# jopohl/urh

Hardware: AMD Instinct MI355X
Metric: Msamples/s IQ->bits (1 GiB complex64 2-FSK per GPU, qad materialised, compact outputs copied to the host) (higher is better)
Workload: dtype f32

## Files before the change

### urh_amd/csrc/costas.hip

```cpp
#include <hip/hip_runtime.h>

#include <algorithm>
#include <atomic>
#include <math.h>
#include <string.h>
#include <type_traits>

#include "cmul.hpp"
#include "common.hpp"
#include "launchers.hpp"
#include "glibc_sincosf.h"

namespace urh {

struct CostasArgs {
    const void *iq; int64_t n; float *out;
    float noise_sqrd, alpha, beta, scale, shift;
    int loop_order;
    int warm;
    const float *d_noise = nullptr;
};
struct CostasState { float freq, phase; };
struct CostasArgsSh : CostasArgs {
    const void *halo_end;
    int64_t origin;
    int64_t lo;
    int64_t start1;
};
template <bool SH> using CostasArgsT = typename std::conditional<SH, CostasArgsSh, CostasArgs>::type;

__device__ __forceinline__ float costas_clamp(float x) {
    float r = (x > 1.0f) ? 1.0f : x;
    r = (x < -1.0f) ? -1.0f : r;
    return r;
}

template <int DT> struct CostasLoad;
template <> struct CostasLoad<URHGPU_DT_F32> { static __device__ __forceinline__ float2 at(const void *p, int64_t i) { return ((const float2 *)p)[i]; } };
template <> struct CostasLoad<URHGPU_DT_I8> { static __device__ __forceinline__ float2 at(const void *p, int64_t i) { const char2 v = ((const char2 *)p)[i]; return make_float2((float)v.x, (float)v.y); } };
template <> struct CostasLoad<URHGPU_DT_U8> { static __device__ __forceinline__ float2 at(const void *p, int64_t i) { const uchar2 v = ((const uchar2 *)p)[i]; return make_float2((float)v.x, (float)v.y); } };
template <> struct CostasLoad<URHGPU_DT_I16> { static __device__ __forceinline__ float2 at(const void *p, int64_t i) { const short2 v = ((const short2 *)p)[i]; return make_float2((float)v.x, (float)v.y); } };
template <> struct CostasLoad<URHGPU_DT_U16> { static __device__ __forceinline__ float2 at(const void *p, int64_t i) { const ushort2 v = ((const ushort2 *)p)[i]; return make_float2((float)v.x, (float)v.y); } };

template <class A>
__device__ __forceinline__ A costas_device_noise(const A &a_in) {
    A a = a_in;
    if (a.d_noise) a.noise_sqrd = *a.d_noise;
    return a;
}
__device__ __forceinline__ bool costas_gated(float2 sm, const CostasArgs &a) { return sm.x * sm.x + sm.y * sm.y <= a.noise_sqrd; }

template <bool UNIT = false, int ORDER = 0>
__device__ __forceinline__ float costas_step(float2 sm, CostasState &st, float &err, const CostasArgs &a) {
    const int loop_order = ORDER ? ORDER : a.loop_order;
    if (costas_gated(sm, a)) return -4.0f;
    const double two_pi = 2 * 3.14159265358979323846;
    const float real_float = UNIT ? sm.x + 0.0f : (sm.x + a.shift) / a.scale, imag_float = UNIT ? sm.y + 0.0f : (sm.y + a.shift) / a.scale;
    const float2 cur = make_float2(real_float + 0.0f * imag_float, 1.0f * imag_float);
    float sn, cs;
    if (urh_sc_abstop12(st.phase) < 0x42f) urh_sincosf_fast(-st.phase, &sn, &cs);
    else { sn = urh_sinf(-st.phase); cs = urh_cosf(-st.phase); }
    const float2 nco = make_float2(cs + 0.0f * sn, 1.0f * sn);
    const float2 z = cmul(nco, cur);
    if (loop_order == 2) {
        err = z.y * z.x;
    } else if (loop_order == 4) {
        const float f1 = z.x > 0.0f ? 1.0f : -1.0f, f2 = z.y > 0.0f ? 1.0f : -1.0f;
        err = f1 * z.y - f2 * z.x;
    }
    err = costas_clamp(err);
    st.freq += a.beta * err;
    st.phase += st.freq + a.alpha * err;
    while ((double)st.phase > two_pi) st.phase = (float)((double)st.phase - two_pi);
    while ((double)st.phase < -two_pi) st.phase = (float)((double)st.phase + two_pi);
    st.freq = costas_clamp(st.freq);
    if (loop_order == 2) return z.x;
    if (loop_order == 4) return (float)(2.0 * (double)z.x + (double)z.y);
    return 0.0f;
}

template <bool UNIT, int ORDER>
__device__ __forceinline__ float costas_step_bf(float2 sm, CostasState &st, float &err, const CostasArgs &a) {
    static_assert(ORDER == 2 || ORDER == 4, "the serial kernel handles the other orders");
    const double two_pi = 2 * 3.14159265358979323846;
    const CostasState old = st;
    const float old_err = err;
    const bool gated = costas_gated(sm, a);
    const float real_float = UNIT ? sm.x + 0.0f : (sm.x + a.shift) / a.scale, imag_float = UNIT ? sm.y + 0.0f : (sm.y + a.shift) / a.scale;
    const float2 cur = make_float2(real_float + 0.0f * imag_float, 1.0f * imag_float);
    const bool in_range = __builtin_fabsf(old.phase) <= __uint_as_float(0x40C90FDBu);
    float sn, cs;
    urh_sincosf_fast(-old.phase, &sn, &cs);
    const float2 nco = make_float2(cs + 0.0f * sn, 1.0f * sn);
    float2 z;
    z.x = nco.x * cur.x - nco.y * cur.y;
    z.y = nco.x * cur.y + nco.y * cur.x;
    const bool rare = !gated && (!in_range || ((z.x != z.x) & (z.y != z.y)));
    float e;
    if (ORDER == 2) e = z.y * z.x;
    else {
        const float f1 = z.x > 0.0f ? 1.0f : -1.0f, f2 = z.y > 0.0f ? 1.0f : -1.0f;
        e = f1 * z.y - f2 * z.x;
    }
    e = costas_clamp(e);
    float freq = old.freq + a.beta * e;
    float phase = old.phase + (freq + a.alpha * e);
    const double d = (double)phase;
    const float wrapped_down = (float)(d - two_pi), wrapped_up = (float)(d + two_pi);
    phase = (d > two_pi) ? wrapped_down : ((d < -two_pi) ? wrapped_up : phase);
    freq = costas_clamp(freq);
    const float out = (ORDER == 2) ? z.x : (float)(2.0 * (double)z.x + (double)z.y);
    if (__builtin_expect(__builtin_amdgcn_ballot_w64(rare) != 0, 0)) {
        st = old; err = old_err;
        return costas_step<UNIT, ORDER>(sm, st, err, a);
    }
    st.freq = gated ? old.freq : freq;
    st.phase = gated ? old.phase : phase;
    err = gated ? old_err : e;
    return gated ? -4.0f : out;
}

constexpr int kCostasTile = 1024;

template <int DT>
__global__ __launch_bounds__(64) void k_costas(const CostasArgs a_in) {
    const CostasArgs a = costas_device_noise(a_in);
    __shared__ float2 s_x[kCostasTile];
    const int lane = threadIdx.x;
    CostasState st{0.0f, 1.5f};
    float err = 0.0f;
    if (lane == 0 && a.n > 0) a.out[0] = -4.0f;
    for (int64_t base = 0; base < a.n; base += kCostasTile) {
        const int tv = (int)((a.n - base < kCostasTile) ? (a.n - base) : kCostasTile);
        __syncthreads();
        for (int u = lane; u < tv; u += 64) s_x[u] = CostasLoad<DT>::at(a.iq, base + u);
        __syncthreads();
        float mine[kCostasTile / 64];
#pragma unroll 1
        for (int g = 0; g < kCostasTile / 64; ++g) {
            float keep = 0.0f;
#pragma unroll 1
            for (int u = 0; u < 64; ++u) {
                const int k = g * 64 + u;
                if (k >= tv || (base + k) == 0) continue;
                const float o = costas_step<DT == URHGPU_DT_F32>(s_x[k], st, err, a);
                if (u == lane) keep = o;
            }
            mine[g] = keep;
        }
#pragma unroll 1
        for (int g = 0; g < kCostasTile / 64; ++g) {
            const int k = g * 64 + lane;
            if (k < tv && base + k != 0) a.out[base + k] = mine[g];
        }
    }
}

#ifndef URH_COSTAS_CHUNK
#define URH_COSTAS_CHUNK 4096
#endif
constexpr int kChunk = URH_COSTAS_CHUNK;
constexpr int kWarmBackFactor = 16;
constexpr int kCkpt = 256;
constexpr int kNumCkpt = kChunk / kCkpt;
constexpr int kMaxCand = 8;

struct SpecBuffers {
    CostasState *S;
    CostasState *E;
    CostasState *CP;
    uint32_t *map;
    CostasState *T;
    int32_t *run_list;
    int32_t *run_count;
    uint8_t *is_rep;
    int32_t *gidx;
    int32_t *ungated;
    CostasState *resume;
    int32_t *stats;
};
struct CostasCtl {
    int64_t c_from;
    int32_t use_seed;
    float seed_freq;
    int32_t done;
    int32_t rounds;
};
__host__ __device__ __forceinline__ CostasCtl *costas_ctl(const SpecBuffers &b) { return (CostasCtl *)(b.stats + 16); }

__device__ __forceinline__ bool same_state(CostasState a, CostasState b) {
    return __float_as_uint(a.freq) == __float_as_uint(b.freq) && __float_as_uint(a.phase) == __float_as_uint(b.phase);
}
__device__ __forceinline__ int64_t chunk_begin(int64_t c) { return 1 + c * (int64_t)kChunk; }

template <bool SH, class A> __device__ __forceinline__ int64_t chunk_begin_of(const A &a, int64_t c) {
    if constexpr (SH) return a.origin + c * (int64_t)kChunk;
    else return chunk_begin(c);
}
template <int DT, bool SH, class A> __device__ __forceinline__ float2 costas_at(const A &a, int64_t i) {
    if constexpr (SH) return CostasLoad<DT>::at(i < 0 ? a.halo_end : a.iq, i);
    else return CostasLoad<DT>::at(a.iq, i);
}
template <bool SH, class A> __device__ __forceinline__ int64_t walk_floor(const A &a) {
    if constexpr (SH) return a.lo;
    else return 1;
}
template <bool SH, class A> __device__ __forceinline__ int64_t loop_start(const A &a) {
    if constexpr (SH) return a.start1;
    else return 1;
}
template <bool SH, class A> __device__ __forceinline__ bool chunk0_exact(const A &a) {
    if constexpr (SH) return a.origin == 1;
    else return true;
}

template <int DT, int ORDER, bool SH = false, bool DEV = false>
__global__ __launch_bounds__(256) void k_costas_spec(const CostasArgsT<SH> a_in, SpecBuffers b, int64_t n_chunks, int K, int64_t c_from,
                                                      int use_seed, float seed_freq) {
    const CostasArgsT<SH> a = costas_device_noise(a_in);
    if constexpr (DEV) {
        if (costas_ctl(b)->done) return;
        c_from = costas_ctl(b)->c_from; use_seed = costas_ctl(b)->use_seed; seed_freq = costas_ctl(b)->seed_freq;
    }
    const int64_t gid = blockIdx.x * 256ll + threadIdx.x;
    const int64_t c = c_from + gid / K;
    const int k = (int)(gid % K);
    if (c >= n_chunks) return;
    const int64_t s0 = chunk_begin_of<SH>(a, c);
    const float spacing = (a.loop_order == 4) ? 1.57079632679489661923f : 3.14159265358979323846f;
    CostasState st{0.0f, 1.5f + (float)(k - K / 2) * spacing};
    float err = 0.0f;
    int64_t p = s0;
    if (c == 0 && chunk0_exact<SH>(a)) {
        st = CostasState{0.0f, 1.5f};
    } else {
        int ungated = 0;
        const int64_t back = (int64_t)kWarmBackFactor * a.warm;
        const int64_t floor = walk_floor<SH>(a);
        while (p > floor && ungated < a.warm && s0 - p < back) {
            float2 g[8];
#pragma unroll
            for (int j = 0; j < 8; ++j) g[j] = costas_at<DT, SH>(a, (p - 1 - j >= floor) ? p - 1 - j : floor);
#pragma unroll
            for (int j = 0; j < 8; ++j) {
                if (p > floor && ungated < a.warm && s0 - p < back) {
                    --p;
                    if (!costas_gated(g[j], a)) ++ungated;
                }
            }
        }
        if (p == loop_start<SH>(a)) {
            st = CostasState{0.0f, 1.5f};
        } else if (use_seed) {
            st.freq = seed_freq;
        } else {
            float ax = 0.0f, ay = 0.0f;
            float2 prev = costas_at<DT, SH>(a, p);
            bool prev_ok = !costas_gated(prev, a);
            const int64_t wend = (p + 512 < s0) ? p + 512 : s0;
            for (int64_t i0 = p + 1; i0 < wend; i0 += 8) {
                float2 g[8];
#pragma unroll
                for (int j = 0; j < 8; ++j) g[j] = costas_at<DT, SH>(a, (i0 + j < wend) ? i0 + j : wend - 1);
#pragma unroll
                for (int j = 0; j < 8; ++j) {
                    if (i0 + j < wend) {
                        const float2 cur = g[j];
                        const bool ok = !costas_gated(cur, a);
                        if (ok && prev_ok) {
                            const float cr = (cur.x + a.shift) / a.scale, ci = (cur.y + a.shift) / a.scale;
                            const float pr = (prev.x + a.shift) / a.scale, pi = (prev.y + a.shift) / a.scale;
                            float dx = cr * pr + ci * pi, dy = ci * pr - cr * pi;
                            float tx = dx * dx - dy * dy, ty = 2.0f * dx * dy;
                            if (a.loop_order == 4) { const float ux = tx * tx - ty * ty, uy = 2.0f * tx * ty; tx = ux; ty = uy; }
                            ax += tx; ay += ty;
                        }
                        prev = cur; prev_ok = ok;
                    }
                }
            }
            if (ax != 0.0f || ay != 0.0f) st.freq = costas_clamp(atan2f(ay, ax) / (float)a.loop_order);
        }
        {
            constexpr int PF = 4;
            float2 cur[PF];
#pragma unroll
            for (int j = 0; j < PF; ++j) cur[j] = costas_at<DT, SH>(a, (p + j < s0) ? p + j : s0 - 1);
            for (int64_t i = p; i < s0; i += PF) {
                float2 nxt[PF];
#pragma unroll
                for (int j = 0; j < PF; ++j) { const int64_t q = i + PF + j; nxt[j] = costas_at<DT, SH>(a, (q < s0) ? q : s0 - 1); }
#pragma unroll
                for (int j = 0; j < PF; ++j) if (i + j < s0) costas_step_bf<DT == URHGPU_DT_F32, ORDER>(cur[j], st, err, a);
#pragma unroll
                for (int j = 0; j < PF; ++j) cur[j] = nxt[j];
            }
        }
    }
    b.S[c * K + k] = st;
    const int lane = threadIdx.x & 63, base = lane - k;
    bool dup = false;
    for (int j = 0; j < K; ++j) {
        CostasState o;
        o.freq = __shfl(st.freq, base + j); o.phase = __shfl(st.phase, base + j);
        if (j < k && same_state(o, st)) dup = true;
    }
    b.is_rep[c * K + k] = dup ? 0 : 1;
    const unsigned long long m = __ballot(!dup);
    int pos = 0;
    if (lane == __builtin_ctzll(m)) pos = atomicAdd(b.run_count, __builtin_popcountll(m));
    pos = __shfl(pos, __builtin_ctzll(m));
    if (!dup) b.run_list[pos + __builtin_popcountll(m & ((1ull << lane) - 1ull))] = (int32_t)(c * K + k);
}

template <int DT, int ORDER, bool SH = false>
__global__ __launch_bounds__(256) void k_costas_run(const CostasArgsT<SH> a_in, SpecBuffers b, int K) {
    const CostasArgsT<SH> a = costas_device_noise(a_in);
    const int64_t gid = blockIdx.x * 256ll + threadIdx.x;
    if (gid >= *b.run_count) return;
    const int64_t ck = b.run_list[gid];
    const int64_t c = ck / K;
    const int k = (int)(ck % K);
    const int64_t s0 = chunk_begin_of<SH>(a, c);
    const int64_t e0 = (s0 + kChunk < a.n) ? s0 + kChunk : a.n;
    CostasState st = b.S[ck];
    float err = 0.0f;
    int ung = 0;
    constexpr int PF = 4;
    float2 cur[PF];
#pragma unroll
    for (int j = 0; j < PF; ++j) cur[j] = CostasLoad<DT>::at(a.iq, (s0 + j < e0) ? s0 + j : e0 - 1);
    for (int64_t i = s0; i < e0; i += PF) {
        float2 nxt[PF];
#pragma unroll
        for (int j = 0; j < PF; ++j) { const int64_t q = i + PF + j; nxt[j] = CostasLoad<DT>::at(a.iq, (q < e0) ? q : e0 - 1); }
#pragma unroll
        for (int j = 0; j < PF; ++j) {
            if (i + j < e0) {
                if (!costas_gated(cur[j], a)) ++ung;
                costas_step_bf<DT == URHGPU_DT_F32, ORDER>(cur[j], st, err, a);
                const int off = (int)(i + j - s0) + 1;
                if (off % kCkpt == 0 && off < kChunk) b.CP[(c * kNumCkpt + (off / kCkpt - 1)) * K + k] = st;
            }
        }
#pragma unroll
        for (int j = 0; j < PF; ++j) cur[j] = nxt[j];
    }
    b.E[ck] = st;
    if (k == 0) b.ungated[c] = ung;
}

template <bool DEV = false>
__global__ __launch_bounds__(256) void k_costas_map(SpecBuffers b, int64_t n_chunks, int K, int64_t c_from) {
    if constexpr (DEV) {
        if (costas_ctl(b)->done) return;
        c_from = costas_ctl(b)->c_from > 1 ? costas_ctl(b)->c_from : 1;
    }
    const int64_t c = c_from + blockIdx.x * 256ll + threadIdx.x;
    if (c >= n_chunks) return;
    uint32_t m = 0xFFFFFFFFu;
    if (c > 0) {
        for (int k = 0; k < K; ++k) {
            int hit = 0xF;
            if (b.is_rep[(c - 1) * K + k]) {
                const CostasState e = b.E[(c - 1) * K + k];
                for (int q = 0; q < K; ++q) if (same_state(e, b.S[c * K + q])) { hit = q; break; }
            }
            m = (m & ~(0xFu << (4 * k))) | ((uint32_t)hit << (4 * k));
        }
    }
    b.map[c] = m;
}

__device__ __forceinline__ uint32_t map_compose(uint32_t later, uint32_t earlier) {
    uint32_t r = 0;
#pragma unroll
    for (int k = 0; k < 8; ++k) {
        const uint32_t mid = (earlier >> (4 * k)) & 0xFu;
        const uint32_t v = (mid == 0xFu) ? 0xFu : ((later >> (4 * mid)) & 0xFu);
        r |= v << (4 * k);
    }
    return r;
}

constexpr int kStitchBlock = 1024;
template <int DT, int ORDER, bool SH = false, bool DEV = false>
__global__ __launch_bounds__(kStitchBlock) void k_costas_stitch(const CostasArgsT<SH> a_in, SpecBuffers b, int64_t n_chunks, int K, int64_t c_from,
                                                                 int allow_break) {
    const CostasArgsT<SH> a = costas_device_noise(a_in);
    if constexpr (DEV) {
        const int done = costas_ctl(b)->done;
        c_from = costas_ctl(b)->c_from > 1 ? costas_ctl(b)->c_from : 1;
        __syncthreads();
        if (done) return;
    }
    __shared__ uint32_t s_wp[kStitchBlock / 64];
    __shared__ int s_fail, s_cand, s_flags;
    __shared__ CostasState s_T;
    __shared__ long long s_c;
    const int tid = threadIdx.x, lane = tid & 63, wave = tid >> 6;
    int cand = -1;
    CostasState T = *b.resume;
    if (!SH && c_from == 1) { cand = 0; if (tid == 0) { b.T[0] = CostasState{0.0f, 1.5f}; b.gidx[0] = 0; } }
    int n_map = 0, n_ckpt = 0, n_serial = 0;
    int64_t stop_at = n_chunks;
    int64_t c = c_from;
    bool map_failed = false;
    bool stop = false;
    while (c < n_chunks && !stop) {
        while (cand >= 0 && c < n_chunks) {
            constexpr int Q = 4;
            if (tid == 0) s_fail = 0x7fffffff;
            const int64_t cc0 = c + (int64_t)Q * tid;
            uint32_t L[Q];
#pragma unroll
            for (int q = 0; q < Q; ++q) {
                const uint32_t m = (cc0 + q < n_chunks) ? b.map[cc0 + q] : 0xFFFFFFFFu;
                L[q] = q ? map_compose(m, L[q - 1]) : m;
            }
            uint32_t P = L[Q - 1];
#pragma unroll
            for (int o = 1; o < 64; o <<= 1) {
                const uint32_t u = __shfl_up(P, o);
                if (lane >= o) P = map_compose(P, u);
            }
            if (lane == 63) s_wp[wave] = P;
            __syncthreads();
            uint32_t X = 0x76543210u;
            for (int w = 0; w < wave; ++w) X = map_compose(s_wp[w], X);
            const uint32_t before = __shfl_up(P, 1);
            if (lane != 0) X = map_compose(before, X);
            uint32_t g[Q], gp[Q];
#pragma unroll
            for (int q = 0; q < Q; ++q) g[q] = (map_compose(L[q], X) >> (4 * cand)) & 0xFu;
            gp[0] = (X >> (4 * cand)) & 0xFu;
#pragma unroll
            for (int q = 1; q < Q; ++q) gp[q] = g[q - 1];
            CostasState Tl[Q];
            int firstq = Q;
#pragma unroll
            for (int q = Q - 1; q >= 0; --q) {
                const int64_t cc = cc0 + q;
                const bool reach = (gp[q] != 0xFu) && (cc < n_chunks);
                Tl[q] = T;
                if (reach) { Tl[q] = b.E[(cc - 1) * K + gp[q]]; b.T[cc] = Tl[q]; b.gidx[cc] = (g[q] == 0xFu) ? -1 : (int32_t)g[q]; }
                if (reach && g[q] == 0xFu) firstq = q;
            }
            if (firstq < Q) atomicMin(&s_fail, tid * Q + firstq);
            __syncthreads();
            const int fail = s_fail;
            const int64_t left = n_chunks - c;
            const int total = (int)(left < (int64_t)kStitchBlock * Q ? left : (int64_t)kStitchBlock * Q);
            const int pos = (fail == 0x7fffffff) ? total - 1 : fail;
            if (tid == pos / Q) {
                const int qq = pos % Q;
                uint32_t gl = g[0];
                CostasState Ts = Tl[0];
#pragma unroll
                for (int q = 1; q < Q; ++q) if (qq == q) { gl = g[q]; Ts = Tl[q]; }
                s_cand = (int)gl; s_T = Ts;
            }
            __syncthreads();
            if (fail == 0x7fffffff) {
                cand = s_cand;
                n_map += total; c += total;
            } else {
                T = s_T;
                n_map += fail; c += fail; cand = -1; map_failed = true;
            }
            __syncthreads();
        }
        if (c >= n_chunks) break;
        if (wave == 0) {
            bool done = false;
            if (!map_failed) {
                if (lane == 0) { b.T[c] = T; b.gidx[c] = -1; }
                const bool hit = lane < K && same_state(T, b.S[c * K + lane]);
                const unsigned long long m = __ballot(hit);
                if (m) {
                    cand = __builtin_ctzll(m);
                    if (lane == 0) b.gidx[c] = cand;
                    ++n_map; ++c;
                    done = true;
                }
            }
            if (!done) {
                map_failed = false;
                if (b.ungated[c] == 0) { ++n_serial; ++c; done = true; }
            }
            if (!done) {
                const int64_t s0 = chunk_begin_of<SH>(a, c);
                const int64_t e0 = (s0 + kChunk < a.n) ? s0 + kChunk : a.n;
                float err = 0.0f;
                CostasState st = T;
                for (int64_t i = s0; i < e0; ++i) {
                    costas_step_bf<DT == URHGPU_DT_F32, ORDER>(CostasLoad<DT>::at(a.iq, i), st, err, a);
                    const int off = (int)(i - s0) + 1;
                    if (off % kCkpt == 0 && off < kChunk) {
                        const bool hit = lane < K && b.is_rep[c * K + lane] && same_state(st, b.CP[(c * kNumCkpt + (off / kCkpt - 1)) * K + lane]);
                        const unsigned long long m = __ballot(hit);
                        if (m) { cand = __builtin_ctzll(m); break; }
                    }
                }
                if (cand >= 0) { ++n_ckpt; ++c; }
                else {
                    ++n_serial;
                    T = st;
                    if (allow_break && b.ungated[c] >= kChunk / 2 && c + 1 < n_chunks) { stop_at = c + 1; stop = true; }
                    else ++c;
                }
            }
            if (lane == 0) { s_c = c; s_cand = cand; s_T = T; s_flags = (map_failed ? 1 : 0) | (stop ? 2 : 0); }
        }
        __syncthreads();
        c = s_c; cand = s_cand; T = s_T; map_failed = (s_flags & 1) != 0; stop = (s_flags & 2) != 0;
        __syncthreads();
    }
    if (tid == 0) {
        b.stats[0] += n_map; b.stats[1] += n_ckpt; b.stats[2] += n_serial; b.stats[3] = (int32_t)stop_at;
        *b.resume = T;
        if constexpr (SH) b.resume[1] = (cand >= 0) ? b.E[(n_chunks - 1) * K + cand] : T;
        if constexpr (DEV) {
            CostasCtl *ctl = costas_ctl(b);
            if (stop_at < n_chunks) { ctl->c_from = stop_at; ctl->use_seed = 1; ctl->seed_freq = T.freq; ctl->rounds += 1; }
            else ctl->done = 1;
            b.stats[4] = ctl->rounds;
        }
    }
}

template <int DT, int ORDER, bool SH = false>
__global__ __launch_bounds__(256) void k_costas_final(const CostasArgsT<SH> a_in, SpecBuffers b, int64_t n_chunks, int K) {
    const CostasArgsT<SH> a = costas_device_noise(a_in);
    const int64_t gid = blockIdx.x * 256ll + threadIdx.x;
    const int64_t c = gid / kNumCkpt;
    const int j = (int)(gid % kNumCkpt);
    if (c >= n_chunks) return;
    if (gid == 0 && a.n > 0 && chunk0_exact<SH>(a)) a.out[0] = -4.0f;
    const int64_t s0 = chunk_begin_of<SH>(a, c);
    const int64_t e0 = (s0 + kChunk < a.n) ? s0 + kChunk : a.n;
    const int g = b.gidx[c];
    int64_t i0 = s0, i1 = e0;
    CostasState st = b.T[c];
    if (g >= 0) {
        i0 = s0 + (int64_t)j * kCkpt;
        i1 = (i0 + kCkpt < e0) ? i0 + kCkpt : e0;
        if (j > 0) st = b.CP[(c * kNumCkpt + (j - 1)) * K + g];
    } else if (j != 0) return;
    float err = 0.0f;
    constexpr int kTileF = 16;
    int64_t i = i0;
    for (; i + kTileF <= i1; i += kTileF) {
        float2 x[kTileF];
#pragma unroll
        for (int u = 0; u < kTileF; ++u) x[u] = CostasLoad<DT>::at(a.iq, i + u);
        float o[kTileF];
#pragma unroll 1
        for (int u = 0; u < kTileF; ++u) {
            float2 xv = x[0];
#pragma unroll
            for (int q = 1; q < kTileF; ++q) if (u == q) xv = x[q];
            const float ov = costas_step_bf<DT == URHGPU_DT_F32, ORDER>(xv, st, err, a);
#pragma unroll
            for (int q = 0; q < kTileF; ++q) if (u == q) o[q] = ov;
        }
#pragma unroll
        for (int u = 0; u < kTileF; ++u) a.out[i + u] = o[u];
    }
    for (; i < i1; ++i) a.out[i] = costas_step_bf<DT == URHGPU_DT_F32, ORDER>(CostasLoad<DT>::at(a.iq, i), st, err, a);
}

constexpr size_t kCtlSlot = 64;
static_assert(sizeof(CostasCtl) <= kCtlSlot, "control block");
size_t costas_scratch_bytes(int64_t n) {
    const int64_t nc = (std::max<int64_t>(n - 1, 0) + kChunk - 1) / kChunk + 1;
    return (size_t)nc * kMaxCand * sizeof(CostasState) * 2 + (size_t)nc * kNumCkpt * kMaxCand * sizeof(CostasState) +
           (size_t)nc * 4 * 3 + (size_t)nc * sizeof(CostasState) + (size_t)nc * kMaxCand * 5 + 3 * 64 + kCtlSlot + 16 * 256;
}

constexpr int kMaxRounds = 24;
std::atomic<long long> g_costas_host_syncs{0};

static SpecBuffers spec_buffers(void *scratch, int64_t nc, int K) {
    char *p = (char *)scratch;
    auto take = [&](size_t bytes) { char *r = p; p += (bytes + 255) & ~size_t(255); return r; };
    SpecBuffers b;
    b.S = (CostasState *)take((size_t)nc * K * sizeof(CostasState));
    b.E = (CostasState *)take((size_t)nc * K * sizeof(CostasState));
    b.CP = (CostasState *)take((size_t)nc * kNumCkpt * K * sizeof(CostasState));
    b.map = (uint32_t *)take((size_t)nc * 4);
    b.T = (CostasState *)take((size_t)nc * sizeof(CostasState));
    b.ungated = (int32_t *)take((size_t)nc * 4);
    b.gidx = (int32_t *)take((size_t)nc * 4);
    b.run_list = (int32_t *)take((size_t)nc * K * 4);
    b.is_rep = (uint8_t *)take((size_t)nc * K);
    b.run_count = (int32_t *)take(64);
    b.resume = (CostasState *)take(64);
    b.stats = (int32_t *)take(64 + kCtlSlot);
    return b;
}
void costas_scratch_layout(int64_t n, int K, int64_t out3[3]) {
    const int64_t nc = (std::max<int64_t>(n - 1, 0) + kChunk - 1) / kChunk;
    const SpecBuffers b = spec_buffers(nullptr, nc, K);
    out3[0] = (int64_t)costas_scratch_bytes(n);
    out3[1] = (int64_t)(uintptr_t)costas_ctl(b) + (int64_t)sizeof(CostasCtl);
    out3[2] = (int64_t)sizeof(CostasCtl);
}

template <int DT, int ORDER>
static int launch_costas_spec(const CostasArgs &a, void *scratch, urhgpu_ctx *ctx);
template <int DT, int ORDER>
static int launch_costas_dev(const CostasArgs &a, void *scratch, urhgpu_ctx *ctx, int rounds, int32_t *h_stats);

constexpr double kEmptyRoundUs = 25.0, kCostasBaseUs = 1800.0, kCostasUsPerChunk = 0.046, kEmptyRoundsShare = 0.10;
static int costas_auto_rounds(int64_t nc) {
    const double fit = kEmptyRoundsShare * (kCostasBaseUs + kCostasUsPerChunk * (double)nc) / kEmptyRoundUs;
    return (int)std::min<double>(kMaxRounds, std::max<double>(2.0, fit));
}

template <int DT>
static int launch_costas_dt(const CostasArgs &a, void *scratch, urhgpu_ctx *ctx) {
    const bool parallel = (a.loop_order == 2 || a.loop_order == 4) && a.n > 2 * kChunk && scratch != nullptr;
    int32_t *h_stats = ctx->costas_stats_next ? ctx->costas_stats_next : (int32_t *)(ctx->h_counts + 12);
    if (!parallel) {
        hipLaunchKernelGGL(k_costas<DT>, dim3(1), dim3(64), 0, ctx->stream, a);
        memset(h_stats, 0, 24);
        return URHGPU_OK;
    }
    if (ctx->tune_costas_dev_rounds >= 0 || ctx->pipelined) {
        const int rounds = ctx->tune_costas_dev_rounds >= 0 ? ctx->tune_costas_dev_rounds : costas_auto_rounds((a.n - 1 + kChunk - 1) / kChunk);
        return a.loop_order == 4 ? launch_costas_dev<DT, 4>(a, scratch, ctx, rounds, h_stats) : launch_costas_dev<DT, 2>(a, scratch, ctx, rounds, h_stats);
    }
    return a.loop_order == 4 ? launch_costas_spec<DT, 4>(a, scratch, ctx) : launch_costas_spec<DT, 2>(a, scratch, ctx);
}

template <int DT, int ORDER>
static int launch_costas_dev(const CostasArgs &a, void *scratch, urhgpu_ctx *ctx, int rounds, int32_t *h_stats) {
    hipStream_t s = ctx->stream;
    const int K = (a.loop_order == 4) ? 8 : 4;
    const int64_t nc = (a.n - 1 + kChunk - 1) / kChunk;
    SpecBuffers b = spec_buffers(scratch, nc, K);
    URH_HIP(hipMemsetAsync(b.stats, 0, 64 + kCtlSlot, s));
    URH_HIP(hipMemsetAsync(b.resume, 0, 64, s));
    const dim3 g_cand((unsigned)((nc * K + 255) / 256)), g_chunk((unsigned)((nc + 255) / 256));
    for (int round = 0; round <= rounds; ++round) {
        URH_HIP(hipMemsetAsync(b.run_count, 0, 4, s));
        hipLaunchKernelGGL((k_costas_spec<DT, ORDER, false, true>), g_cand, dim3(256), 0, s, a, b, nc, K, (int64_t)0, 0, 0.0f);
        hipLaunchKernelGGL((k_costas_run<DT, ORDER>), g_cand, dim3(256), 0, s, a, b, K);
        hipLaunchKernelGGL(k_costas_map<true>, g_chunk, dim3(256), 0, s, b, nc, K, (int64_t)1);
        hipLaunchKernelGGL((k_costas_stitch<DT, ORDER, false, true>), dim3(1), dim3(kStitchBlock), 0, s, a, b, nc, K, (int64_t)1, round < rounds ? 1 : 0);
    }
    hipLaunchKernelGGL((k_costas_final<DT, ORDER>), dim3((unsigned)((nc * kNumCkpt + 255) / 256)), dim3(256), 0, s, a, b, nc, K);
    URH_HIP(hipGetLastError());
    URH_HIP(hipMemcpyAsync(h_stats, b.stats, 20, hipMemcpyDeviceToHost, s));
    return URHGPU_OK;
}

template <int DT, int ORDER>
static int launch_costas_spec(const CostasArgs &a, void *scratch, urhgpu_ctx *ctx) {
    hipStream_t s = ctx->stream;
    const int K = (a.loop_order == 4) ? 8 : 4;
    const int64_t nc = (a.n - 1 + kChunk - 1) / kChunk;
    SpecBuffers b = spec_buffers(scratch, nc, K);
    URH_HIP(hipMemsetAsync(b.stats, 0, 64, s));
    URH_HIP(hipMemsetAsync(b.resume, 0, 64, s));
    int64_t c_from = 0;
    int use_seed = 0;
    float seed_freq = 0.0f;
    int32_t *h = (int32_t *)(ctx->h_counts + 12);
    int rounds = 0;
    for (int round = 0;; ++round) {
        const int64_t todo = nc - c_from;
        URH_HIP(hipMemsetAsync(b.run_count, 0, 4, s));
        hipLaunchKernelGGL((k_costas_spec<DT, ORDER>), dim3((unsigned)((todo * K + 255) / 256)), dim3(256), 0, s, a, b, nc, K, c_from, use_seed,
                           seed_freq);
        hipLaunchKernelGGL((k_costas_run<DT, ORDER>), dim3((unsigned)((todo * K + 255) / 256)), dim3(256), 0, s, a, b, K);
        hipLaunchKernelGGL(k_costas_map<false>, dim3((unsigned)((todo + 255) / 256)), dim3(256), 0, s, b, nc, K, std::max<int64_t>(c_from, 1));
        hipLaunchKernelGGL((k_costas_stitch<DT, ORDER>), dim3(1), dim3(kStitchBlock), 0, s, a, b, nc, K, std::max<int64_t>(c_from, 1),
                           round < kMaxRounds ? 1 : 0);
        URH_HIP(hipGetLastError());
        URH_HIP(hipMemcpyAsync(h, b.stats, 20, hipMemcpyDeviceToHost, s));
        URH_HIP(hipMemcpyAsync(h + 6, b.resume, 8, hipMemcpyDeviceToHost, s));
        URH_HIP(hipStreamSynchronize(s));
        ++g_costas_host_syncs;
        center_note_wait();
        const int64_t stop_at = h[3];
        if (stop_at >= nc) break;
        c_from = stop_at;
        use_seed = 1;
        memcpy(&seed_freq, h + 6, 4);
        rounds = round + 1;
    }
    h[4] = rounds;
    hipLaunchKernelGGL((k_costas_final<DT, ORDER>), dim3((unsigned)((nc * kNumCkpt + 255) / 256)), dim3(256), 0, s, a, b, nc, K);
    return URHGPU_OK;
}

static int costas_warm(float bandwidth) {
    const double want = 40.0 / std::max(1e-3, std::min(1.0, (double)fabsf(bandwidth)));
    int w = 256;
    while (w < want && w < 8192) w *= 2;
    return w;
}

static int costas_args(const urhgpu_params *p, CostasArgs &a) {
    a.noise_sqrd = p->noise_threshold * p->noise_threshold;
    const float bandwidth = p->costas_loop_bandwidth;
    const float damping = (float)(sqrt(2.0) / 2.0);
    const double den = (1.0 + ((2.0 * (double)damping) * (double)bandwidth)) + (double)(bandwidth * bandwidth);
    a.alpha = (float)(((4.0 * (double)damping) * (double)bandwidth) / den);
    a.beta = (float)(((4.0 * (double)bandwidth) * (double)bandwidth) / den);
    switch (p->dtype) {
        case URHGPU_DT_I8: a.scale = 127.5f; a.shift = 0.5f; break;
        case URHGPU_DT_U8: a.scale = 127.5f; a.shift = -127.5f; break;
        case URHGPU_DT_I16: a.scale = 32767.5f; a.shift = 0.5f; break;
        case URHGPU_DT_U16: a.scale = 65535.0f; a.shift = -32767.5f; break;
        case URHGPU_DT_F32: a.scale = 1.0f; a.shift = 0.0f; break;
        default: return URHGPU_ERR_DTYPE;
    }
    a.warm = costas_warm(bandwidth);
    int order = p->mod_order > 0 ? p->mod_order : (1 << p->bits_per_symbol);
    if (order > 4) order = 4;
    a.loop_order = order;
    return URHGPU_OK;
}

int launch_costas(urhgpu_ctx *ctx, const void *d_iq, int64_t n, const urhgpu_params *p, float *d_qad, void *scratch, const float *d_noise) {
    CostasArgs a;
    a.iq = d_iq; a.n = n; a.out = d_qad; a.d_noise = d_noise;
    URH_TRY(costas_args(p, a));
    switch (p->dtype) {
        case URHGPU_DT_I8: return launch_costas_dt<URHGPU_DT_I8>(a, scratch, ctx);
        case URHGPU_DT_U8: return launch_costas_dt<URHGPU_DT_U8>(a, scratch, ctx);
        case URHGPU_DT_I16: return launch_costas_dt<URHGPU_DT_I16>(a, scratch, ctx);
        case URHGPU_DT_U16: return launch_costas_dt<URHGPU_DT_U16>(a, scratch, ctx);
        default: return launch_costas_dt<URHGPU_DT_F32>(a, scratch, ctx);
    }
}


int64_t costas_halo_samples(const urhgpu_params *p) { return (int64_t)kWarmBackFactor * costas_warm(p->costas_loop_bandwidth); }

constexpr int kSumBlock = 1024;
__global__ __launch_bounds__(kSumBlock) void k_costas_shard_summary(SpecBuffers b, int64_t n_chunks, int K, uint32_t *out) {
    __shared__ uint32_t s_wp[kSumBlock / 64];
    __shared__ unsigned long long s_ung;
    const int tid = threadIdx.x, lane = tid & 63, wave = tid >> 6;
    if (tid == 0) s_ung = 0;
    __syncthreads();
    unsigned long long ung = 0;
    for (int64_t c = tid; c < n_chunks; c += kSumBlock) ung += (uint32_t)b.ungated[c];
    atomicAdd(&s_ung, ung);
    uint32_t R = 0x76543210u;
    constexpr int Q = 4;
    for (int64_t c0 = 1; c0 < n_chunks; c0 += (int64_t)kSumBlock * Q) {
        const int64_t cc0 = c0 + (int64_t)Q * tid;
        uint32_t P = 0x76543210u;
#pragma unroll
        for (int q = 0; q < Q; ++q) if (cc0 + q < n_chunks) P = map_compose(b.map[cc0 + q], P);
#pragma unroll
        for (int o = 1; o < 64; o <<= 1) {
            const uint32_t u = __shfl_up(P, o);
            if (lane >= o) P = map_compose(P, u);
        }
        if (lane == 63) s_wp[wave] = P;
        __syncthreads();
        for (int w = 0; w < kSumBlock / 64; ++w) R = map_compose(s_wp[w], R);
        __syncthreads();
    }
    __syncthreads();
    if (tid < kCostasSummaryBytes / 4) {
        const int64_t last = (n_chunks - 1) * K;
        uint32_t v = 0;
        if (tid < 16) {
            const int k = tid >> 1;
            if (k < K) { const CostasState s = b.S[k]; v = __float_as_uint((tid & 1) ? s.phase : s.freq); }
        } else if (tid < 32) {
            const int k = (tid - 16) >> 1;
            if (k < K && b.is_rep[last + k]) { const CostasState e = b.E[last + k]; v = __float_as_uint((tid & 1) ? e.phase : e.freq); }
        } else if (tid == 32) {
            v = R;
        } else if (tid == 33) {
            for (int k = 0; k < K; ++k) v |= b.is_rep[k] ? (1u << k) : 0u;
        } else if (tid == 34) {
            v = (s_ung == 0) ? 1u : 0u;
        } else if (tid == 35) {
            v = (uint32_t)K;
        } else if (tid < 38) {
            v = (uint32_t)((uint64_t)n_chunks >> (32 * (tid - 36)));
        } else {
            v = (uint32_t)(s_ung >> (32 * (tid - 38)));
        }
        out[tid] = v;
    }
}

__global__ void k_costas_set_state(CostasState *dst, uint32_t freq_bits, uint32_t phase_bits) {
    uint32_t *d = (uint32_t *)dst;
    d[0] = freq_bits; d[1] = phase_bits;
}

static int costas_shard_args(const CostasShard &cs, CostasArgsSh &a, int64_t &nc) {
    a.iq = cs.iq; a.n = cs.n; a.out = cs.out;
    URH_TRY(costas_args(&cs.p, a));
    if (a.loop_order != 2 && a.loop_order != 4) return URHGPU_ERR_UNSUPPORTED;
    a.halo_end = cs.halo_end; a.origin = cs.origin; a.lo = cs.lo; a.start1 = cs.start1;
    nc = (cs.n - cs.origin + kChunk - 1) / kChunk;
    return URHGPU_OK;
}

template <int DT, int ORDER>
static int costas_shard_spec_t(urhgpu_ctx *ctx, const CostasArgsSh &a, int64_t nc, void *scratch, void *d_summary) {
    hipStream_t s = ctx->stream;
    const int K = (ORDER == 4) ? 8 : 4;
    const SpecBuffers b = spec_buffers(scratch, nc, K);
    URH_HIP(hipMemsetAsync(b.stats, 0, 64, s));
    URH_HIP(hipMemsetAsync(b.resume, 0, 64, s));
    URH_HIP(hipMemsetAsync(b.run_count, 0, 4, s));
    const unsigned g = (unsigned)((nc * K + 255) / 256);
    hipLaunchKernelGGL((k_costas_spec<DT, ORDER, true>), dim3(g), dim3(256), 0, s, a, b, nc, K, (int64_t)0, 0, 0.0f);
    hipLaunchKernelGGL((k_costas_run<DT, ORDER, true>), dim3(g), dim3(256), 0, s, a, b, K);
    hipLaunchKernelGGL(k_costas_map<false>, dim3((unsigned)((nc + 255) / 256)), dim3(256), 0, s, b, nc, K, (int64_t)1);
    hipLaunchKernelGGL(k_costas_shard_summary, dim3(1), dim3(kSumBlock), 0, s, b, nc, K, (uint32_t *)d_summary);
    URH_HIP(hipGetLastError());
    return URHGPU_OK;
}

template <int DT, int ORDER>
static int costas_shard_resolve_t(urhgpu_ctx *ctx, const CostasArgsSh &a, int64_t nc, void *scratch, uint32_t freq_bits, uint32_t phase_bits,
                                  void *d_end) {
    hipStream_t s = ctx->stream;
    const int K = (ORDER == 4) ? 8 : 4;
    const SpecBuffers b = spec_buffers(scratch, nc, K);
    hipLaunchKernelGGL(k_costas_set_state, dim3(1), dim3(1), 0, s, b.resume, freq_bits, phase_bits);
    int64_t c_from = 0;
    float seed_freq = 0.0f;
    int32_t *h = (int32_t *)(ctx->h_counts + 12);
    int rounds = 0;
    for (int round = 0;; ++round) {
        if (round > 0) {
            const int64_t todo = nc - c_from;
            URH_HIP(hipMemsetAsync(b.run_count, 0, 4, s));
            hipLaunchKernelGGL((k_costas_spec<DT, ORDER, true>), dim3((unsigned)((todo * K + 255) / 256)), dim3(256), 0, s, a, b, nc, K, c_from, 1,
                               seed_freq);
            hipLaunchKernelGGL((k_costas_run<DT, ORDER, true>), dim3((unsigned)((todo * K + 255) / 256)), dim3(256), 0, s, a, b, K);
            hipLaunchKernelGGL(k_costas_map<false>, dim3((unsigned)((todo + 255) / 256)), dim3(256), 0, s, b, nc, K, c_from);
        }
        hipLaunchKernelGGL((k_costas_stitch<DT, ORDER, true>), dim3(1), dim3(kStitchBlock), 0, s, a, b, nc, K, c_from,
                           round < kMaxRounds ? 1 : 0);
        URH_HIP(hipGetLastError());
        URH_HIP(hipMemcpyAsync(h, b.stats, 20, hipMemcpyDeviceToHost, s));
        URH_HIP(hipMemcpyAsync(h + 6, b.resume, 8, hipMemcpyDeviceToHost, s));
        URH_HIP(hipStreamSynchronize(s));
        ++g_costas_host_syncs;
        center_note_wait();
        const int64_t stop_at = h[3];
        if (stop_at >= nc) break;
        c_from = stop_at;
        memcpy(&seed_freq, h + 6, 4);
        rounds = round + 1;
    }
    h[4] = rounds;
    if (d_end) URH_HIP(hipMemcpyAsync(d_end, b.resume + 1, 8, hipMemcpyDeviceToDevice, s));
    hipLaunchKernelGGL((k_costas_final<DT, ORDER, true>), dim3((unsigned)((nc * kNumCkpt + 255) / 256)), dim3(256), 0, s, a, b, nc, K);
    URH_HIP(hipGetLastError());
    return URHGPU_OK;
}

#define URH_COSTAS_SHARD_DISPATCH(FN, ...)                                                                                       \
    switch (cs.p.dtype) {                                                                                                        \
        case URHGPU_DT_I8: return a.loop_order == 4 ? FN<URHGPU_DT_I8, 4>(__VA_ARGS__) : FN<URHGPU_DT_I8, 2>(__VA_ARGS__);        \
        case URHGPU_DT_U8: return a.loop_order == 4 ? FN<URHGPU_DT_U8, 4>(__VA_ARGS__) : FN<URHGPU_DT_U8, 2>(__VA_ARGS__);        \
        case URHGPU_DT_I16: return a.loop_order == 4 ? FN<URHGPU_DT_I16, 4>(__VA_ARGS__) : FN<URHGPU_DT_I16, 2>(__VA_ARGS__);     \
        case URHGPU_DT_U16: return a.loop_order == 4 ? FN<URHGPU_DT_U16, 4>(__VA_ARGS__) : FN<URHGPU_DT_U16, 2>(__VA_ARGS__);     \
        case URHGPU_DT_F32: return a.loop_order == 4 ? FN<URHGPU_DT_F32, 4>(__VA_ARGS__) : FN<URHGPU_DT_F32, 2>(__VA_ARGS__);     \
        default: return URHGPU_ERR_DTYPE;                                                                                        \
    }

int launch_costas_shard_spec(urhgpu_ctx *ctx, const CostasShard &cs, void *d_summary) {
    CostasArgsSh a;
    int64_t nc = 0;
    URH_TRY(costas_shard_args(cs, a, nc));
    URH_COSTAS_SHARD_DISPATCH(costas_shard_spec_t, ctx, a, nc, cs.scratch, d_summary)
}

int launch_costas_shard_resolve(urhgpu_ctx *ctx, const CostasShard &cs, uint32_t freq_bits, uint32_t phase_bits, void *d_end) {
    CostasArgsSh a;
    int64_t nc = 0;
    URH_TRY(costas_shard_args(cs, a, nc));
    URH_COSTAS_SHARD_DISPATCH(costas_shard_resolve_t, ctx, a, nc, cs.scratch, freq_bits, phase_bits, d_end)
}
#undef URH_COSTAS_SHARD_DISPATCH

__global__ __launch_bounds__(256) void k_test_sincosf_fast(unsigned long long *mismatches) {
    unsigned long long bad = 0;
    for (uint64_t u = blockIdx.x * 256ull + threadIdx.x; u < 2ull * 0x42f00000ull; u += (uint64_t)gridDim.x * 256ull) {
        const uint32_t bits = (u < 0x42f00000ull) ? (uint32_t)u : ((uint32_t)(u - 0x42f00000ull) | 0x80000000u);
        const float y = __uint_as_float(bits);
        float sn, cs;
        urh_sincosf_fast(y, &sn, &cs);
        if (__float_as_uint(sn) != __float_as_uint(urh_sinf(y)) || __float_as_uint(cs) != __float_as_uint(urh_cosf(y))) ++bad;
    }
    if (bad) atomicAdd(mismatches, bad);
}
void launch_test_sincosf_fast(unsigned long long *d_mismatches, hipStream_t s) {
    hipLaunchKernelGGL(k_test_sincosf_fast, dim3(256 * 32), dim3(256), 0, s, d_mismatches);
}

}
```

Measured before the change: 496,700.

## Split Costas warm-up backward walk and frequency seed across the K hypothesis lanes

Result: no change. 496,500 (-0.0%).

```diff
diff --git a/urh_amd/csrc/costas.hip b/urh_amd/csrc/costas.hip
--- a/urh_amd/csrc/costas.hip
+++ b/urh_amd/csrc/costas.hip
@@ -214,6 +214,21 @@
     else return true;
 }
 
+__device__ __forceinline__ int nth_set_bit(uint64_t m, int n) {
+    int pos = 0;
+#pragma unroll
+    for (int w = 32; w; w >>= 1) {
+        const int low = __builtin_popcountll(m & ((1ull << w) - 1ull));
+        const bool skip = n > low;
+        n = skip ? n - low : n; m = skip ? m >> w : m; pos = skip ? pos + w : pos;
+    }
+    return pos;
+}
+template <int DT> __device__ __forceinline__ float2 seed_scaled(float2 sm, float shift, float inv_scale) {
+    if constexpr (DT == URHGPU_DT_F32) return sm;
+    else return make_float2((sm.x + shift) * inv_scale, (sm.y + shift) * inv_scale);
+}
+
 template <int DT, int ORDER, bool SH = false, bool DEV = false>
 __global__ __launch_bounds__(256) void k_costas_spec(const CostasArgsT<SH> a_in, SpecBuffers b, int64_t n_chunks, int K, int64_t c_from,
                                                       int use_seed, float seed_freq) {
@@ -226,6 +241,8 @@
     const int64_t c = c_from + gid / K;
     const int k = (int)(gid % K);
     if (c >= n_chunks) return;
+    constexpr int KK = (ORDER == 4) ? 8 : 4;
+    const int lane = threadIdx.x & 63, base = lane - k;
     const int64_t s0 = chunk_begin_of<SH>(a, c);
     const float spacing = (a.loop_order == 4) ? 1.57079632679489661923f : 3.14159265358979323846f;
     CostasState st{0.0f, 1.5f + (float)(k - K / 2) * spacing};
@@ -237,16 +254,25 @@
         int ungated = 0;
         const int64_t back = (int64_t)kWarmBackFactor * a.warm;
         const int64_t floor = walk_floor<SH>(a);
-        while (p > floor && ungated < a.warm && s0 - p < back) {
+        const int64_t lim = (s0 - back > floor) ? s0 - back : floor;
+        while (p > lim && ungated < a.warm) {
+            const int room = (p - lim > 8 * KK) ? 8 * KK : (int)(p - lim);
             float2 g[8];
 #pragma unroll
-            for (int j = 0; j < 8; ++j) g[j] = costas_at<DT, SH>(a, (p - 1 - j >= floor) ? p - 1 - j : floor);
+            for (int j = 0; j < 8; ++j) { const int t = j * KK + k; g[j] = costas_at<DT, SH>(a, p - 1 - ((t < room) ? t : room - 1)); }
+            uint64_t seen = 0;
 #pragma unroll
             for (int j = 0; j < 8; ++j) {
-                if (p > floor && ungated < a.warm && s0 - p < back) {
-                    --p;
-                    if (!costas_gated(g[j], a)) ++ungated;
-                }
+                const unsigned long long bal = __ballot(j * KK + k < room && !costas_gated(g[j], a));
+                seen |= ((bal >> base) & ((1ull << KK) - 1ull)) << (j * KK);
+            }
+            const int have = __builtin_popcountll(seen), need = a.warm - ungated;
+            if (have < need) {
+                ungated += have;
+                p -= room;
+            } else {
+                ungated = a.warm;
+                p -= 1 + nth_set_bit(seen, need);
             }
         }
         if (p == loop_start<SH>(a)) {
@@ -255,30 +281,36 @@
             st.freq = seed_freq;
         } else {
             float ax = 0.0f, ay = 0.0f;
-            float2 prev = costas_at<DT, SH>(a, p);
-            bool prev_ok = !costas_gated(prev, a);
             const int64_t wend = (p + 512 < s0) ? p + 512 : s0;
-            for (int64_t i0 = p + 1; i0 < wend; i0 += 8) {
-                float2 g[8];
-#pragma unroll
-                for (int j = 0; j < 8; ++j) g[j] = costas_at<DT, SH>(a, (i0 + j < wend) ? i0 + j : wend - 1);
-#pragma unroll
-                for (int j = 0; j < 8; ++j) {
-                    if (i0 + j < wend) {
-                        const float2 cur = g[j];
-                        const bool ok = !costas_gated(cur, a);
-                        if (ok && prev_ok) {
-                            const float cr = (cur.x + a.shift) / a.scale, ci = (cur.y + a.shift) / a.scale;
-                            const float pr = (prev.x + a.shift) / a.scale, pi = (prev.y + a.shift) / a.scale;
-                            float dx = cr * pr + ci * pi, dy = ci * pr - cr * pi;
-                            float tx = dx * dx - dy * dy, ty = 2.0f * dx * dy;
-                            if (a.loop_order == 4) { const float ux = tx * tx - ty * ty, uy = 2.0f * tx * ty; tx = ux; ty = uy; }
-                            ax += tx; ay += ty;
-                        }
+            const int n_pairs = (wend > p + 1) ? (int)(wend - (p + 1)) : 0;
+            const int share = (n_pairs + KK - 1) / KK;
+            const int first = k * share;
+            const int mine = (first + share <= n_pairs) ? share : ((n_pairs > first) ? n_pairs - first : 0);
+            if (mine > 0) {
+                const float inv_scale = 1.0f / a.scale;
+                const int64_t i_lo = p + 1 + first;
+                float2 raw = costas_at<DT, SH>(a, i_lo - 1);
+                bool prev_ok = !costas_gated(raw, a);
+                float2 prev = seed_scaled<DT>(raw, a.shift, inv_scale);
+                for (int o = 0; o < mine; o += 8) {
+                    float2 g[8];
+#pragma unroll
+                    for (int j = 0; j < 8; ++j) g[j] = costas_at<DT, SH>(a, i_lo + ((o + j < mine) ? o + j : mine - 1));
+#pragma unroll
+                    for (int j = 0; j < 8; ++j) {
+                        const bool ok = !costas_gated(g[j], a);
+                        const float2 cur = seed_scaled<DT>(g[j], a.shift, inv_scale);
+                        float dx = cur.x * prev.x + cur.y * prev.y, dy = cur.y * prev.x - cur.x * prev.y;
+                        float tx = dx * dx - dy * dy, ty = 2.0f * dx * dy;
+                        if (ORDER == 4) { const float ux = tx * tx - ty * ty, uy = 2.0f * tx * ty; tx = ux; ty = uy; }
+                        const bool take = ok && prev_ok && o + j < mine;
+                        ax += take ? tx : 0.0f; ay += take ? ty : 0.0f;
                         prev = cur; prev_ok = ok;
                     }
                 }
             }
+#pragma unroll
+            for (int m = 1; m < KK; m <<= 1) { ax += __shfl_xor(ax, m); ay += __shfl_xor(ay, m); }
             if (ax != 0.0f || ay != 0.0f) st.freq = costas_clamp(atan2f(ay, ax) / (float)a.loop_order);
         }
         {
@@ -298,7 +330,6 @@
         }
     }
     b.S[c * K + k] = st;
-    const int lane = threadIdx.x & 63, base = lane - k;
     bool dup = false;
     for (int j = 0; j < K; ++j) {
         CostasState o;
```
